# ChaissonLab/LRA

Hardware: AMD Instinct MI355X
Metric: aligned Gbp/s, 30 kb ONT vs GRCh38 (MapRead_lowacc end to end incl. SAM text), per job (higher is better)
Workload: dtype int32

## Files before the change

### lra_amd/csrc/indel_refine.hip

```cpp
#include "common.h"
#include "scan.h"
#include <algorithm>
#include <stdlib.h>

int lra_aog_launch_device(lra_ctx* ctx, int n, const char* d_qseq, const char* d_tseq, const uint64_t* d_q_off,
                          const int32_t* d_q_len, const uint64_t* d_t_off, const int32_t* d_t_len, const int32_t* d_k,
                          int m, int mm, int indel, int32_t* d_score, int32_t* d_nblocks, int32_t* d_blocks,
                          const uint64_t* d_block_off, int32_t* d_status);

namespace {

constexpr int BAD = -999999999;
constexpr int NEG = -2000000000;
enum { C_DIAG = 0, C_LEFT = 1, C_DOWN = 2, C_BOUND = 3, C_DELCLOSE = 4, C_INSCLOSE = 5, C_DONE = 6 };

__device__ __forceinline__ void wave_sync() {
  __builtin_amdgcn_fence(__ATOMIC_RELEASE, "workgroup");
  __builtin_amdgcn_wave_barrier();
  __builtin_amdgcn_fence(__ATOMIC_ACQUIRE, "workgroup");
}

__device__ __forceinline__ void wave_sync_lds() {
  __builtin_amdgcn_fence(__ATOMIC_RELEASE, "wavefront");
  __builtin_amdgcn_wave_barrier();
// ... 58 lines not shown
  auto get = [&](long i, long& q, long& t, long& l) {
    if (i == ovIdx) { q = ovQ; t = ovT; l = ovL; } else getRaw(i, q, t, l);
  };
  long startBlock = 0, endBlock = 0;
  while (endBlock < nB) {
    long q0, t0, l0;
    get(startBlock, q0, t0, l0);
    long qStart = q0, tStart = t0;
    long qPos = q0 + l0, tPos = t0 + l0;
    int tGap = 0, qGap = 0;
    long nq, nt, nl;
    if (endBlock < nB - 1) { get(endBlock + 1, nq, nt, nl); tGap = (int)(nt - tPos); qGap = (int)(nq - qPos); }
    long el = l0, eq = q0, et = t0;
    while (endBlock < nB - 1 && qGap < maxGap && tGap < maxGap && (startBlock == endBlock || el < 100)) {
      endBlock++;
      get(endBlock, eq, et, el);
      qPos = eq + el; tPos = et + el;
      if (endBlock + 1 < nB - 1) { get(endBlock + 1, nq, nt, nl); tGap = (int)(nt - tPos); qGap = (int)(nq - qPos); }
    }
    bool usedAlt = false;
    long altQ = 0, altT = 0, altL = 0;
    if (endBlock == startBlock) {
      pass(q0, t0, l0);
    } else {
      long fq = q0, ft = t0, fl = l0;
      if (l0 > maxGap) {
        long advanced = l0 - maxGap;
        pass(q0, t0, advanced);
        fq = q0 + advanced; ft = t0 + advanced; fl = maxGap;
        qStart += advanced; tStart += advanced;
      }
      long ll = el;
      if (el > maxGap) {
        usedAlt = true;
        altQ = eq + maxGap; altT = et + maxGap; altL = el - maxGap;
        ll = maxGap;
        qPos = eq + maxGap; tPos = et + maxGap;
      }
      const long qEnd = eq + ll, tEnd = et + ll;
      const long tLen = tPos - tStart;
      const long tSeqLen = tEnd - tStart, qSeqLen = qEnd - qStart;
      const bool aog = (tSeqLen < k || qSeqLen < k);
      if (EMIT) {
        const uint64_t s = so + nseg;
        A.s_aln[s] = a; A.s_kind[s] = aog ? 1 : 0;
        A.s_qStart[s] = (int)qStart; A.s_tStart[s] = (int)tStart; A.s_qEnd[s] = (int)qEnd; A.s_tEnd[s] = (int)tEnd;
        A.s_b0[s] = (int)startBlock; A.s_b1[s] = (int)endBlock;
        A.s_first[3 * s] = (int)fq; A.s_first[3 * s + 1] = (int)ft; A.s_first[3 * s + 2] = (int)fl;
        A.s_lastLen[s] = (int)ll;
        A.s_rows[s] = aog ? 0 : (uint64_t)(tLen > 0 ? tLen : 0);
        A.s_isAog[s] = aog ? 1u : 0u;
        A.i_kind[io + nitem] = 1; A.i_data[3 * (io + nitem)] = (int)(nseg);
      }
      nitem++; nseg++;
    }
    if (!usedAlt) endBlock++;
    else { ovIdx = endBlock; ovQ = altQ; ovT = altT; ovL = altL; }
    startBlock = endBlock;
  }
  if (!EMIT) { A.a_nseg[a] = nseg; A.a_nitem[a] = nitem; A.a_status[a] = 0; }
}

struct __attribute__((aligned(16))) Row { int S, E; unsigned int C; int T; };

constexpr int CB = 32;
constexpr int MAXW = 1024;

struct BandArgs {
  uint64_t n_seg, n_task;
  const int32_t* s_aln; const int32_t* s_kind; const int32_t* s_qStart; const int32_t* s_qEnd; const int32_t* s_tStart;
  const int32_t* s_b0; const int32_t* s_b1; const int32_t* s_first; const int32_t* s_lastLen;
  const uint64_t* s_rows; const uint64_t* s_row_off;
  const int32_t* ab; const uint64_t* block_off;
  const char* tseq; const uint64_t* t_off;
  int k;
  Row* rows;
  uint64_t* s_cells; int32_t* s_status; int32_t* s_width; uint64_t* s_tmpcap;
  uint32_t* s_nchunk; const uint64_t* chunk_off; uint32_t* task_seg; int32_t* chunkT; int32_t* chunkQ;
};

struct SegBlocks {
  const int32_t* ab; long b0, b1; int fq, ft, fl, lastLen;
  __device__ __forceinline__ void get(long b, long& q, long& t, long& l) const {
    if (b == b0) { q = fq; t = ft; l = fl; }
    else { q = ab[3 * b]; t = ab[3 * b + 1]; l = (b == b1) ? lastLen : ab[3 * b + 2]; }
  }
};
__device__ __forceinline__ SegBlocks seg_blocks(const BandArgs& B, uint64_t s) {
  SegBlocks v;
  const int a = B.s_aln[s];
  v.ab = B.ab + 3 * (B.block_off[a] + 2 * (uint64_t)a);
  v.b0 = B.s_b0[s]; v.b1 = B.s_b1[s];
  v.fq = B.s_first[3 * s]; v.ft = B.s_first[3 * s + 1]; v.fl = B.s_first[3 * s + 2]; v.lastLen = B.s_lastLen[s];
  return v;
}
struct BlockStep { int bqGap, btGap; long blockLength, rows, advq; };
__device__ __forceinline__ BlockStep block_step(const SegBlocks& sb, long b, long bq, long bt, long bl, long& nq2, long& nt2, long& nl2) {
  BlockStep st; st.bqGap = 0; st.btGap = 0; st.blockLength = bl; nq2 = nt2 = nl2 = 0;
  if (b < sb.b1) {
    sb.get(b + 1, nq2, nt2, nl2);
    st.bqGap = (int)(nq2 - (bq + bl)); st.btGap = (int)(nt2 - (bt + bl));
    if (st.bqGap > 0 && st.btGap > 0) { int c = min(st.bqGap, st.btGap); st.bqGap -= c; st.btGap -= c; st.blockLength += c; }
  }
  const long body = st.blockLength > 0 ? st.blockLength : 0;
  st.rows = body + (st.btGap > st.bqGap && st.btGap > 0 ? st.btGap : 0);
  st.advq = body + (st.bqGap > st.btGap && st.bqGap > 0 ? st.bqGap : 0);
  return st;
}

__global__ void ir_band_nchunk(BandArgs B) {
  const uint64_t s = (uint64_t)blockIdx.x * blockDim.x + threadIdx.x;
  if (s >= B.n_seg) return;
  B.s_nchunk[s] = (B.s_kind[s] != 0) ? 0u : (uint32_t)((B.s_b1[s] - B.s_b0[s] + 1 + CB - 1) / CB);
}
__global__ void ir_band_tasks(BandArgs B) {
  const uint64_t s = (uint64_t)blockIdx.x * blockDim.x + threadIdx.x;
  if (s >= B.n_seg) return;
  const uint64_t lo = B.chunk_off[s], hi = B.chunk_off[s + 1];
  for (uint64_t x = lo; x < hi; x++) B.task_seg[x] = (uint32_t)s;
  if (hi - lo <= 1) B.s_status[s] = 0;
}

__global__ void __launch_bounds__(64) ir_band_prep(BandArgs B) {
  const uint64_t s = blockIdx.x;
  const int lane = threadIdx.x;
  const uint64_t co = B.chunk_off[s];
  if (B.chunk_off[s + 1] - co <= 1) return;
  const SegBlocks sb = seg_blocks(B, s);
  const long nb = sb.b1 - sb.b0 + 1;
  long long carryT = 0, carryQ = 0;
  for (long base = 0; base < nb; base += 64) {
    const long i = base + lane;
    long long r = 0, q = 0;
    if (i < nb) {
      long bq, bt, bl, nq2, nt2, nl2;
      sb.get(sb.b0 + i, bq, bt, bl);
      const BlockStep st = block_step(sb, sb.b0 + i, bq, bt, bl, nq2, nt2, nl2);
      r = st.rows; q = st.advq;
    }
    long long ir = r, iq = q;
    for (int d = 1; d < 64; d <<= 1) {
      long long orr = __shfl_up(ir, d), oq = __shfl_up(iq, d);
      if (lane >= d) { ir += orr; iq += oq; }
    }
    if (i < nb && i > 0 && (i % CB) == 0) {
      B.chunkT[co + i / CB] = (int32_t)(carryT + ir - r);
      B.chunkQ[co + i / CB] = (int32_t)(sb.fq + carryQ + iq - q);
    }
    carryT += __shfl(ir, 63); carryQ += __shfl(iq, 63);
  }
  if (lane == 0) B.s_status[s] = (carryT != (long long)B.s_rows[s]) ? 1 : 0;
}

template <int RS>
__global__ void __launch_bounds__(64) ir_band_chunk(BandArgs B) {
  __shared__ int ringS[RS * 64], ringE[RS * 64];
  const int lane = threadIdx.x;
  const uint64_t x = (uint64_t)blockIdx.x * 64 + lane;
  if (x >= B.n_task) return;
  const uint64_t s = B.task_seg[x];
  const uint64_t co = B.chunk_off[s];
  const long c = (long)(x - co), nch = (long)(B.chunk_off[s + 1] - co);
  const bool multi = nch > 1, lastChunk = (c == nch - 1);
  if (multi && B.s_status[s] != 0) return;
  const long tLen = (long)B.s_rows[s];
  const SegBlocks sb = seg_blocks(B, s);
  const long qStart = B.s_qStart[s], qEnd = B.s_qEnd[s];
  const int k = B.k;
  Row* rows = B.rows + B.s_row_off[s];
  int status = 0;
#define RG(arr, r) arr[(int)((r) & (RS - 1)) * 64 + lane]
  for (int z = 0; z < RS; z++) { ringS[z * 64 + lane] = -1; ringE[z * 64 + lane] = -1; }
  const long bFirst = sb.b0 + c * CB, bLast = min(sb.b1, bFirst + CB - 1);
  const long T0 = c > 0 ? B.chunkT[co + c] : 0;
  long from = c;
  while (from > 0) { from--; if (from == 0 || T0 - B.chunkT[co + from] >= 2 * (long)k - 1) break; }
  const long ownLo = c > 0 ? T0 - k + 1 : 0, thr = T0 - 2 * (long)k + 1;
  long q = from > 0 ? B.chunkQ[co + from] : sb.fq;
  long tOff = from > 0 ? B.chunkT[co + from] : 0;
  auto flush = [&](long r) {
    if (r >= 0 && r < tLen) {
      if (r >= ownLo) { int2 v; v.x = RG(ringS, r); v.y = RG(ringE, r); *(int2*)&rows[r] = v; }
      RG(ringS, r) = -1; RG(ringE, r) = -1;
    }
  };
  long bq, bt, bl;
  sb.get(sb.b0 + from * CB, bq, bt, bl);
  bool live = (c == 0);
  int eMin = -1;
  long sHi = -1;
  for (long b = sb.b0 + from * CB; b <= bLast && !(status & 1); b++) {
    long nq2, nt2, nl2;
    const BlockStep st = block_step(sb, b, bq, bt, bl, nq2, nt2, nl2);
    if (!live) {
      if (b < bFirst && tOff + st.rows <= thr) { tOff += st.rows; q += st.advq; bq = nq2; bt = nt2; bl = nl2; continue; }
      live = true;
    }
    for (long bi = 0; bi < st.blockLength; bi++) {
      if (tOff >= tLen) { status |= 1; break; }
      int newE;
      {
        int lo = (int)max(q - k, qStart);
        int cs = RG(ringS, tOff), ce = RG(ringE, tOff);
        RG(ringS, tOff) = (cs == -1) ? lo : min(cs, lo);
        newE = ce;
        if (ce == -1 || ce < q + k) { newE = (int)min(qEnd - 1, q + k); RG(ringE, tOff) = newE; }
      }
      if (newE < eMin) eMin = newE;
      if (q > eMin) {
        int m = 0x7fffffff;
        for (int ki = 0; ki < k; ki++)
          if (tOff - ki >= 0) { int e = RG(ringE, tOff - ki); if (e < q) { e = (int)q; RG(ringE, tOff - ki) = e; } m = min(m, e); }
        eMin = m;
      }
      if (sHi < tOff) sHi = tOff;
      for (long r = sHi + 1; r <= tOff + k - 1 && r < tLen; r++) RG(ringS, r) = (int)q;
      if (sHi < tOff + k - 1) sHi = tOff + k - 1;
      tOff++; q++;
      flush(tOff - k);
    }
    if (st.bqGap > st.btGap) {
      for (int qi = 0; qi < st.bqGap; qi++, q++)
        for (int ki = 0; ki < k; ki++) {
          if (tOff - ki >= 0 && tOff - ki < tLen) { if (RG(ringE, tOff - ki) < q) RG(ringE, tOff - ki) = (int)q; }
          if (tOff + ki < tLen) { int v = RG(ringS, tOff + ki); if (v == 0 || v > q) RG(ringS, tOff + ki) = (int)q; }
        }
    }
    if (st.btGap > st.bqGap) {
      for (int ti = 0; ti < st.btGap; ti++) {
        if (tOff >= tLen) { status |= 1; break; }
        const int e = (int)min(qEnd - 1, q + k);
        RG(ringS, tOff) = (int)max(q - k, qStart); RG(ringE, tOff) = e;
        if (e < eMin) eMin = e;
        if (sHi < tOff) sHi = tOff;
        tOff++;
        flush(tOff - k);
      }
    }
    bq = nq2; bt = nt2; bl = nl2;
  }
  if (lastChunk) for (long r = max(0L, tOff - k + 1); r < tLen; r++) flush(r);
#undef RG
  if (!multi) { if (tOff != tLen) status |= 1; B.s_status[s] = status; }
}

__global__ void __launch_bounds__(64) ir_band_scan(BandArgs B) {
  const uint64_t s = blockIdx.x;
  const int lane = threadIdx.x;
  if (B.s_kind[s] != 0) { if (lane == 0) { B.s_cells[s] = 0; B.s_status[s] = 0; B.s_width[s] = 0; B.s_tmpcap[s] = 0; } return; }
  int status = B.s_status[s];
  const long tLen = (long)B.s_rows[s];
  Row* rows = B.rows + B.s_row_off[s];
  unsigned long long cells = 0;
  int width = 0;
  if (!status && tLen > 0) {
    int run = 0x7fffffff;
    for (long base = ((tLen - 1) / 64) * 64; base >= 0; base -= 64) {
      const long r = base + lane;
      const int own = (r < tLen) ? rows[r].S : 0x7fffffff;
      int v = own;
      for (int d = 1; d < 64; d <<= 1) { int o = __shfl_down(v, d); if (lane + d < 64) v = min(v, o); }
      v = min(v, run);
      if (r < tLen && v != own) rows[r].S = v;
      run = __shfl(v, 0);
    }
    const int a = B.s_aln[s];
    const unsigned char* tb = (const unsigned char*)B.tseq + B.t_off[a] + B.s_tStart[s];
    int runE = -0x7fffffff;
    for (long base = 0; base < tLen; base += 64) {
      const long r = base + lane;
      Row w; w.S = 0; w.E = -0x7fffffff; w.C = 0; w.T = 0;
      if (r < tLen) w = rows[r];
      int e = w.E;
      for (int d = 1; d < 64; d <<= 1) { int o = __shfl_up(e, d); if (lane >= d) e = max(e, o); }
      e = max(e, runE);
      runE = __shfl(e, 63);
      int len = (r < tLen) ? e - w.S + 1 : 0;
      if (r < tLen) {
        if (len < 1 || w.S < 0) status |= 1;
        else if (len > MAXW) status |= 4;
        width = max(width, len);
      }
      const unsigned long long l = (unsigned long long)max(len, 0);
      unsigned long long inc = l;
      for (int d = 1; d < 64; d <<= 1) { unsigned long long o = __shfl_up(inc, d); if (lane >= d) inc += o; }
      if (r < tLen) { w.E = e; w.C = (unsigned int)(cells + inc - l); w.T = tb[r]; rows[r] = w; }
      cells += __shfl(inc, 63);
    }
    for (int o = 32; o > 0; o >>= 1) { status |= __shfl_xor(status, o); width = max(width, __shfl_xor(width, o)); }
  }
  if (lane == 0) {
    B.s_cells[s] = status ? 0 : cells;
    B.s_status[s] = status;
    B.s_width[s] = status ? 0 : width;
    B.s_tmpcap[s] = status ? 0 : (uint64_t)(tLen + ((long)B.s_qEnd[s] - B.s_qStart[s]) + 2);
  }
}

constexpr int FILL_BINS = 128;
template <bool EMIT>
__global__ void ir_classify(uint64_t n_seg, const int32_t* __restrict__ s_kind, const int32_t* __restrict__ s_status, const int32_t* __restrict__ s_width,
                            const uint64_t* __restrict__ s_rows, int* bins, uint32_t* list) {
  const uint64_t s = (uint64_t)blockIdx.x * blockDim.x + threadIdx.x;
  const int lane = threadIdx.x & 63;
  int bin = -1;
  if (s < n_seg && s_kind[s] == 0 && s_status[s] == 0) {
    const int w = s_width[s];
    const uint32_t r = (uint32_t)min((unsigned long long)s_rows[s], 0x7fffffffULL);
    bin = (w <= 16 ? 0 : w <= 32 ? 1 : w <= 64 ? 2 : 3) * 32 + (r ? __clz(r) : 31);
  }
  const unsigned long long below = (lane == 0) ? 0ULL : (~0ULL >> (64 - lane));
  unsigned long long todo = __ballot(bin >= 0);
  while (todo) {
    const int leader = __ffsll((long long)todo) - 1;
    const int b = __shfl(bin, leader);
    const unsigned long long m = __ballot(bin == b);
    int base = 0;
    if (lane == leader) base = atomicAdd(&bins[b], __popcll(m));
    base = __shfl(base, leader);
    if (EMIT && bin == b) list[base + __popcll(m & below)] = (uint32_t)s;
    todo &= ~m;
  }
}

struct FillArgs {
  uint64_t n_seg;
  const int32_t* s_aln; const uint64_t* s_rows; const uint64_t* s_row_off; const uint64_t* s_cell_off;
  const Row* rows;
  const char* qseq; const uint64_t* q_off; const int32_t* q_len;
  int match, mismatch, g;
  unsigned char* path;
  const uint32_t* list; int* cursor;
};

__device__ __forceinline__ bool is_bound(long row, int c, int len) { return c == len - 1 || (row > 0 && c == 0); }

__device__ __forceinline__ int shr1(int x, int fill) { return __builtin_amdgcn_update_dpp(fill, x, 0x138, 0xf, 0xf, false); }
template <int G>
__device__ __forceinline__ int scan_max(int w) {
  w = max(w, __builtin_amdgcn_update_dpp(NEG, w, 0x111, 0xf, 0xf, false));
  w = max(w, __builtin_amdgcn_update_dpp(NEG, w, 0x112, 0xf, 0xf, false));
  w = max(w, __builtin_amdgcn_update_dpp(NEG, w, 0x114, 0xf, 0xf, false));
  w = max(w, __builtin_amdgcn_update_dpp(NEG, w, 0x118, 0xf, 0xf, false));
  if (G >= 32) w = max(w, __builtin_amdgcn_update_dpp(NEG, w, 0x142, 0xa, 0xf, false));
  if (G >= 64) w = max(w, __builtin_amdgcn_update_dpp(NEG, w, 0x143, 0xc, 0xf, false));
  return w;
}

template <int G>
__global__ void __launch_bounds__(64) ir_fill(FillArgs F) {
  constexpr int GP = 64 / G;
  constexpr int CLS = (G == 16) ? 0 : (G == 32) ? 1 : 2;
  const int lane = threadIdx.x;
  const int c = lane % G, gbase = lane - c;
  const int g = F.g, go = 2 * F.g + 1;
  const long listEnd = F.cursor[4 + CLS];
  const uint32_t* list = F.list;
  long ti = -1, tLen = 0;
  const Row* rows = nullptr; const unsigned char* qb = nullptr; unsigned char* P = nullptr;
  long chunkBase = 0, qLast = 0;
  Row chunk; chunk.S = chunk.E = chunk.T = 0; chunk.C = 0;
  int W0 = 0, qlo = 0, qhi = 0, qnext = 0;
  int prevM = BAD, prevD = BAD, prevS = 0, prevLen = 0;
  bool done = false;
  auto ldq = [&](long idx) -> int { return qb[idx < qLast ? idx : qLast]; };
  while (true) {
    if (!done && ti < 0) {
      long x = 0;
      if (c == 0) x = atomicAdd(&F.cursor[CLS], 1);
      x = __shfl(x, gbase);
      if (x < listEnd) {
        const uint64_t s = list[x];
        const int a = F.s_aln[s];
        tLen = (long)F.s_rows[s];
        rows = F.rows + F.s_row_off[s];
        qb = (const unsigned char*)F.qseq + F.q_off[a];
        qLast = (long)F.q_len[a] - 1;
        P = F.path + F.s_cell_off[s];
        ti = 0; chunkBase = 0;
        if (c < tLen) chunk = rows[c];
        W0 = rows[0].S;
        qlo = ldq((long)W0 + c); qhi = ldq((long)W0 + G + c); qnext = ldq((long)W0 + 2 * G + c);
      } else done = true;
    }
    if (__ballot(!done) == 0ULL) break;
    if (!done && ti - chunkBase == G) { chunkBase = ti; if (ti + c < tLen) chunk = rows[ti + c]; }
    const int src = gbase + (int)((ti - chunkBase) & (G - 1));
    const int S = __shfl(chunk.S, src), E = __shfl(chunk.E, src), tch = __shfl(chunk.T, src);
    const unsigned int C = __shfl(chunk.C, src);
    while (!done && S - W0 >= G) { W0 += G; qlo = qhi; qhi = qnext; qnext = ldq((long)W0 + 2 * G + c); }
    const int j = S - W0 + c;
    const int q1 = __shfl(qlo, gbase + (j & (G - 1))), q2 = __shfl(qhi, gbase + (j & (G - 1)));
    const int qch = (j < G) ? q1 : q2;
    const int len = E - S + 1;
    const bool lastRow = (ti == tLen - 1);
    const int off = S - prevS;
// ... 460 lines not shown
  int st = 0;
  for (uint64_t s = seg_off[a]; s < seg_off[a + 1]; s++) {
    if (s_kind[s] == 0) { int x = s_status[s]; if (x & 1) st |= LRA_ST_OOB_SLOT; if (x & 2) st |= LRA_ST_NO_TERMINATION; if (x & 4) st |= LRA_ST_RANGE; }
    else st |= p_status[s_aog_idx[s]];
  }
  a_status[a] = st;
}

__global__ void ir_item_aln(int n_aln, const uint64_t* item_off, int32_t* i_aln) {
  int a = blockIdx.x * blockDim.x + threadIdx.x;
  if (a >= n_aln) return;
  for (uint64_t i = item_off[a]; i < item_off[a + 1]; i++) i_aln[i] = a;
}

__global__ void ir_aog_setup(uint64_t n_seg, const int32_t* s_kind, const int32_t* s_aln, const uint64_t* s_aog_off ,
                             const int32_t* s_qStart, const int32_t* s_tStart, const int32_t* s_qEnd, const int32_t* s_tEnd,
                             const uint64_t* q_off, const uint64_t* t_off, int k, uint32_t* s_aog_idx, uint64_t* p_q_off, int32_t* p_q_len,
                             uint64_t* p_t_off, int32_t* p_t_len, int32_t* p_k, uint32_t* p_cap) {
  uint64_t s = (uint64_t)blockIdx.x * blockDim.x + threadIdx.x;
  if (s >= n_seg) return;
  if (s_kind[s] != 1) { s_aog_idx[s] = 0; return; }
  uint32_t p = (uint32_t)s_aog_off[s];
  s_aog_idx[s] = p;
  int a = s_aln[s];
  p_q_off[p] = q_off[a] + (uint64_t)s_qStart[s]; p_q_len[p] = s_qEnd[s] - s_qStart[s];
  p_t_off[p] = t_off[a] + (uint64_t)s_tStart[s]; p_t_len[p] = s_tEnd[s] - s_tStart[s];
  p_k[p] = k;
  p_cap[p] = (uint32_t)(min(p_q_len[p], p_t_len[p]) + 1);
}


struct Arena {
  char* base; size_t cap, used;
  template <typename T> T* get(size_t n) {
    size_t bytes = (n * sizeof(T) + 255) & ~(size_t)255;
    if (used + bytes > cap) return nullptr;
    T* p = (T*)(base + used);
    used += bytes;
    return p;
  }
};

}

template <typename CT>
static void scan(lra_ctx* ctx, long n, const CT* c, uint64_t* off) {
  (void)lra_exclusive_scan<CT>(ctx, n, c, off);
}

static int d2h(lra_ctx* ctx, void* dst, const void* src, size_t bytes) {
  LRA_HIP_CHECK(ctx, hipMemcpyAsync(dst, src, bytes, hipMemcpyDeviceToHost, ctx->stream));
  LRA_HIP_CHECK(ctx, hipStreamSynchronize(ctx->stream));
  return LRA_OK;
}

extern "C" int lra_indel_refine_batch(lra_ctx* ctx, int n_aln, const int32_t* d_blocks_in, const uint64_t* d_block_off, uint64_t n_blocks_in,
                                      const char* d_qseq, const uint64_t* d_q_off, const int32_t* d_q_len, const char* d_tseq,
                                      const uint64_t* d_t_off, const int64_t* d_t_len, int refine_band, int match, int mismatch,
                                      int indel, int end_align, lra_refine_result* out) {
  if (!ctx || !out || n_aln < 0) return LRA_ERR_INVALID;
  if (refine_band < 2 || refine_band > 64) return lra_set_err(ctx, LRA_ERR_INVALID, "refine_band must be 2..64");
  if (indel >= 0) return lra_set_err(ctx, LRA_ERR_INVALID, "indel score must be negative");
  memset(out, 0, sizeof(*out));
  if (n_aln == 0) return LRA_OK;
  LRA_HIP_CHECK(ctx, hipSetDevice(ctx->device));
  hipStream_t st = ctx->stream;
  const size_t nA = (size_t)n_aln, nBk = (size_t)n_blocks_in + 2 * nA;
  const size_t perAln = ((nA * 4 + 255) & ~(size_t)255) * 3 + (((nA + 1) * 8 + 255) & ~(size_t)255) * 3;
  char* baseP = (char*)lra_ensure(ctx, 70, perAln + 4096);
  if (!baseP) return LRA_ERR_NOMEM;
  Arena ap{baseP, perAln + 4096, 0};
  IRArgs A;
  memset(&A, 0, sizeof A);
  A.n_aln = n_aln; A.blocks_in = d_blocks_in; A.block_off = d_block_off;
  A.qseq = d_qseq; A.q_off = d_q_off; A.q_len = d_q_len; A.tseq = d_tseq; A.t_off = d_t_off; A.t_len = d_t_len;
  A.k = refine_band; A.match = match; A.mismatch = mismatch; A.indel = indel; A.endAlign = end_align;
  A.a_nseg = ap.get<uint32_t>(nA); A.a_nitem = ap.get<uint32_t>(nA); A.a_status = ap.get<int32_t>(nA);
  uint64_t* seg_off = ap.get<uint64_t>(nA + 1); uint64_t* item_off = ap.get<uint64_t>(nA + 1); uint64_t* out_block_off = ap.get<uint64_t>(nA + 1);
  if (!out_block_off) return lra_set_err(ctx, LRA_ERR_NOMEM, "arena accounting");
  A.seg_off = seg_off; A.item_off = item_off;
  const int nbA = (n_aln + SEG_LANES - 1) / SEG_LANES;
  lra_time_begin(ctx, "ir_segment");
  hipLaunchKernelGGL(ir_segment<false>, dim3(nbA), dim3(64), 0, st, A);
  lra_time_end(ctx);
  scan(ctx, (long)n_aln, A.a_nseg, seg_off);
  scan(ctx, (long)n_aln, A.a_nitem, item_off);
  uint64_t n_seg = 0, n_item = 0;
  if (d2h(ctx, &n_seg, seg_off + n_aln, 8) || d2h(ctx, &n_item, item_off + n_aln, 8)) return LRA_ERR_HIP;
  const size_t capSeg = (size_t)n_seg + 1, capItem = (size_t)n_item + 1;
  size_t needA = 0;
  auto add = [&](size_t n, size_t sz) { needA += ((n * sz + 255) & ~(size_t)255); };
  add(3 * nBk, 4);
  for (int i = 0; i < 8; i++) add(capSeg, 4);
  add(3 * capSeg, 4); add(capSeg, 4); add(capSeg, 8); add(capSeg, 4);
  add(capSeg + 1, 8); add(capSeg + 1, 8); add(capSeg, 8); add(capSeg + 1, 8); add(capSeg, 4);
  add(capSeg, 4); add(capSeg, 4); add(capSeg, 8); add(capSeg + 1, 8); add(capSeg, 4); add(capSeg + 1, 8);
  add(capSeg, 4); add(FILL_BINS + 8, 4);
  add(capItem, 4); add(3 * capItem, 4); add(capItem, 4); add(capItem, 4); add(capItem + 1, 8);
  add(capSeg, 8); add(capSeg, 4); add(capSeg, 8); add(capSeg, 4); add(capSeg, 4); add(capSeg, 4); add(capSeg + 1, 8);
  add(capSeg, 4); add(capSeg, 4); add(capSeg, 4);
  add(capSeg, 4); add(capSeg + 1, 8);
  char* baseA = (char*)lra_scratch(ctx, 2, needA + 4096);
  if (!baseA) return LRA_ERR_NOMEM;
  Arena ar{baseA, needA + 4096, 0};
  A.ab = ar.get<int32_t>(3 * nBk);
  A.s_aln = ar.get<int32_t>(capSeg); A.s_kind = ar.get<int32_t>(capSeg); A.s_qStart = ar.get<int32_t>(capSeg); A.s_tStart = ar.get<int32_t>(capSeg);
  A.s_qEnd = ar.get<int32_t>(capSeg); A.s_tEnd = ar.get<int32_t>(capSeg); A.s_b0 = ar.get<int32_t>(capSeg); A.s_b1 = ar.get<int32_t>(capSeg);
  A.s_first = ar.get<int32_t>(3 * capSeg); A.s_lastLen = ar.get<int32_t>(capSeg); A.s_rows = ar.get<uint64_t>(capSeg); A.s_isAog = ar.get<uint32_t>(capSeg);
  uint64_t* s_row_off = ar.get<uint64_t>(capSeg + 1); uint64_t* s_aog_off = ar.get<uint64_t>(capSeg + 1);
  uint64_t* s_cells = ar.get<uint64_t>(capSeg); uint64_t* s_cell_off = ar.get<uint64_t>(capSeg + 1); int32_t* s_status = ar.get<int32_t>(capSeg);
  uint32_t* s_nblk = ar.get<uint32_t>(capSeg); int32_t* s_width = ar.get<int32_t>(capSeg); uint64_t* s_tmpcap = ar.get<uint64_t>(capSeg);
  uint64_t* s_tmp_off = ar.get<uint64_t>(capSeg + 1); uint32_t* s_aog_idx = ar.get<uint32_t>(capSeg); uint64_t* s_out_off = ar.get<uint64_t>(capSeg + 1);
  uint32_t* fill_lists = ar.get<uint32_t>(capSeg); int* fill_counts = ar.get<int>(FILL_BINS + 8);
  A.i_kind = ar.get<int32_t>(capItem); A.i_data = ar.get<int32_t>(3 * capItem);
  int32_t* i_aln = ar.get<int32_t>(capItem); uint32_t* i_count = ar.get<uint32_t>(capItem); uint64_t* i_out_off = ar.get<uint64_t>(capItem + 1);
  uint64_t* p_q_off = ar.get<uint64_t>(capSeg); int32_t* p_q_len = ar.get<int32_t>(capSeg); uint64_t* p_t_off = ar.get<uint64_t>(capSeg);
  int32_t* p_t_len = ar.get<int32_t>(capSeg); int32_t* p_k = ar.get<int32_t>(capSeg); uint32_t* p_cap = ar.get<uint32_t>(capSeg);
  uint64_t* p_block_off = ar.get<uint64_t>(capSeg + 1);
  int32_t* p_score = ar.get<int32_t>(capSeg); int32_t* p_nblocks = ar.get<int32_t>(capSeg); int32_t* p_status = ar.get<int32_t>(capSeg);
  uint32_t* s_nchunk = ar.get<uint32_t>(capSeg); uint64_t* chunk_off = ar.get<uint64_t>(capSeg + 1);
  if (!chunk_off) return lra_set_err(ctx, LRA_ERR_NOMEM, "arena accounting");
  lra_time_begin(ctx, "ir_segment");
  hipLaunchKernelGGL(ir_segment<true>, dim3(nbA), dim3(64), 0, st, A);
  lra_time_end(ctx);
  hipLaunchKernelGGL(ir_item_aln, dim3((n_aln + 255) / 256), dim3(256), 0, st, n_aln, item_off, i_aln);
  uint64_t n_rows = 0, n_aog = 0, n_cells = 0;
  const int32_t* tmp_blocks = nullptr;
  if (n_seg) {
    scan(ctx, (long)n_seg, A.s_rows, s_row_off);
    scan(ctx, (long)n_seg, A.s_isAog, s_aog_off);
    if (d2h(ctx, &n_rows, s_row_off + n_seg, 8) || d2h(ctx, &n_aog, s_aog_off + n_seg, 8)) return LRA_ERR_HIP;
    Row* rows = (Row*)lra_ensure(ctx, 0, (n_rows + 1) * sizeof(Row));
    if (!rows) return LRA_ERR_NOMEM;
    BandArgs B;
    B.n_seg = n_seg; B.s_aln = A.s_aln; B.s_kind = A.s_kind; B.s_qStart = A.s_qStart; B.s_qEnd = A.s_qEnd; B.s_tStart = A.s_tStart;
    B.s_b0 = A.s_b0; B.s_b1 = A.s_b1; B.s_first = A.s_first; B.s_lastLen = A.s_lastLen; B.s_rows = A.s_rows; B.s_row_off = s_row_off;
    B.ab = A.ab; B.block_off = d_block_off; B.tseq = d_tseq; B.t_off = d_t_off; B.k = refine_band; B.rows = rows;
    B.s_cells = s_cells; B.s_status = s_status; B.s_width = s_width; B.s_tmpcap = s_tmpcap;
    const unsigned gridL = (unsigned)((n_seg + 63) / 64);
    const unsigned gridS = (unsigned)((n_seg + 255) / 256);
    lra_time_begin(ctx, "ir_band");
    B.s_nchunk = s_nchunk; B.chunk_off = chunk_off; B.n_task = 0; B.task_seg = nullptr; B.chunkT = nullptr; B.chunkQ = nullptr;
    hipLaunchKernelGGL(ir_band_nchunk, dim3(gridS), dim3(256), 0, st, B);
    scan(ctx, (long)n_seg, s_nchunk, chunk_off);
    uint64_t n_task = 0;
    if (d2h(ctx, &n_task, chunk_off + n_seg, 8)) return LRA_ERR_HIP;
    uint32_t* task_seg = (uint32_t*)lra_ensure(ctx, 54, (n_task + 1) * 4);
    int32_t* chunk_tq = (int32_t*)lra_ensure(ctx, 55, (n_task + 1) * 8);
    if (!task_seg || !chunk_tq) return LRA_ERR_NOMEM;
    B.n_task = n_task; B.task_seg = task_seg; B.chunkT = chunk_tq; B.chunkQ = chunk_tq + n_task + 1;
    hipLaunchKernelGGL(ir_band_tasks, dim3(gridS), dim3(256), 0, st, B);
    hipLaunchKernelGGL(ir_band_prep, dim3((unsigned)n_seg), dim3(64), 0, st, B);
    if (n_task) {
      const unsigned gridT = (unsigned)((n_task + 63) / 64);
      if (refine_band <= 8) hipLaunchKernelGGL(ir_band_chunk<16>, dim3(gridT), dim3(64), 0, st, B);
      else if (refine_band <= 32) hipLaunchKernelGGL(ir_band_chunk<64>, dim3(gridT), dim3(64), 0, st, B);
      else hipLaunchKernelGGL(ir_band_chunk<128>, dim3(gridT), dim3(64), 0, st, B);
    }
    hipLaunchKernelGGL(ir_band_scan, dim3((unsigned)n_seg), dim3(64), 0, st, B);
    lra_time_end(ctx);
    scan(ctx, (long)n_seg, s_cells, s_cell_off);
    scan(ctx, (long)n_seg, s_tmpcap, s_tmp_off);
    uint64_t n_tmp = 0;
    if (d2h(ctx, &n_cells, s_cell_off + n_seg, 8) || d2h(ctx, &n_tmp, s_tmp_off + n_seg, 8)) return LRA_ERR_HIP;
    const size_t pathBytes = (n_cells + 256 + 255) & ~(size_t)255;
    unsigned char* path = (unsigned char*)lra_ensure(ctx, 12, pathBytes + (n_tmp + 1) * 12 + 256);
    if (!path) return LRA_ERR_NOMEM;
    int32_t* tmpb = (int32_t*)(path + pathBytes);
    tmp_blocks = tmpb;
    int h_bins[FILL_BINS], h_start[FILL_BINS], h_cursor[8] = {0, 0, 0, 0, 0, 0, 0, 0};
    LRA_HIP_CHECK(ctx, hipMemsetAsync(fill_counts, 0, FILL_BINS * 4, st));
    hipLaunchKernelGGL(ir_classify<false>, dim3((unsigned)((n_seg + 255) / 256)), dim3(256), 0, st, n_seg, A.s_kind, s_status, s_width, A.s_rows, fill_counts, fill_lists);
    if (d2h(ctx, h_bins, fill_counts, FILL_BINS * 4)) return LRA_ERR_HIP;
    { int run = 0; for (int b = 0; b < FILL_BINS; b++) { h_start[b] = run; run += h_bins[b]; if ((b & 31) == 0) h_cursor[b / 32] = h_start[b]; if ((b & 31) == 31) h_cursor[4 + b / 32] = run; } }
    LRA_HIP_CHECK(ctx, hipMemcpyAsync(fill_counts, h_start, FILL_BINS * 4, hipMemcpyHostToDevice, st));
    hipLaunchKernelGGL(ir_classify<true>, dim3((unsigned)((n_seg + 255) / 256)), dim3(256), 0, st, n_seg, A.s_kind, s_status, s_width, A.s_rows, fill_counts, fill_lists);
    int* fill_cursor = fill_counts + FILL_BINS;
    LRA_HIP_CHECK(ctx, hipMemcpyAsync(fill_cursor, h_cursor, 32, hipMemcpyHostToDevice, st));
    FillArgs F;
    F.n_seg = n_seg; F.s_aln = A.s_aln; F.s_rows = A.s_rows; F.s_row_off = s_row_off; F.s_cell_off = s_cell_off; F.rows = rows;
    F.qseq = d_qseq; F.q_off = d_q_off; F.q_len = d_q_len; F.match = match; F.mismatch = mismatch; F.g = indel; F.path = path;
    F.list = fill_lists; F.cursor = fill_cursor;
    const unsigned cap_grid = (unsigned)ctx->num_cu * 32;
    if (getenv("LRA_IR_DBG")) {
      const int hc[4] = {h_cursor[4] - h_cursor[0], h_cursor[5] - h_cursor[1], h_cursor[6] - h_cursor[2], h_cursor[7] - h_cursor[3]};
      fprintf(stderr, "[ir] n_seg %llu n_rows %llu n_cells %llu n_task %llu n_item %llu fill classes 16/32/64/wide: %d %d %d %d\n",
              (unsigned long long)n_seg, (unsigned long long)n_rows, (unsigned long long)n_cells, (unsigned long long)n_task,
              (unsigned long long)n_item, hc[0], hc[1], hc[2], hc[3]);
    }
    lra_time_begin(ctx, "ir_fill");
    const uint64_t n16 = (uint64_t)(h_cursor[4] - h_cursor[0]), n32 = (uint64_t)(h_cursor[5] - h_cursor[1]), n64 = (uint64_t)(h_cursor[6] - h_cursor[2]);
    const uint64_t nWide = (uint64_t)(h_cursor[7] - h_cursor[3]);
    if (n16) hipLaunchKernelGGL(ir_fill_cols<1>, dim3((unsigned)std::min<uint64_t>((n16 + 3) / 4, cap_grid)), dim3(64), 0, lra_side_fork(ctx, 1), F);
    if (n64) hipLaunchKernelGGL(ir_fill<64>, dim3((unsigned)std::min<uint64_t>(n64, cap_grid)), dim3(64), 0, lra_side_fork(ctx, 2), F);
    if (nWide) hipLaunchKernelGGL(ir_fill_wide, dim3((unsigned)std::min<uint64_t>(nWide, cap_grid)), dim3(64), 0, lra_side_fork(ctx, 3), F);
    if (n32) hipLaunchKernelGGL(ir_fill_cols<2>, dim3((unsigned)std::min<uint64_t>((n32 + 3) / 4, cap_grid)), dim3(64), 0, st, F);
    if (n16) lra_side_join(ctx, 1);
    if (n64) lra_side_join(ctx, 2);
    if (nWide) lra_side_join(ctx, 3);
    lra_time_end(ctx);
    TraceArgs T;
    T.n_seg = n_seg; T.s_kind = A.s_kind; T.s_tStart = A.s_tStart; T.s_rows = A.s_rows; T.s_row_off = s_row_off;
    T.s_cells = s_cells; T.s_cell_off = s_cell_off; T.s_status = s_status; T.rows = rows; T.path = path;
    T.s_nblk = s_nblk; T.s_tmp_off = s_tmp_off; T.tmp_blocks = tmpb;
    lra_time_begin(ctx, "ir_trace");
    hipLaunchKernelGGL(ir_trace_wave, dim3((unsigned)n_seg), dim3(64), 0, st, T);
    lra_time_end(ctx);
    if (n_aog) {
      hipLaunchKernelGGL(ir_aog_setup, dim3((unsigned)((n_seg + 255) / 256)), dim3(256), 0, st, n_seg, A.s_kind, A.s_aln, s_aog_off, A.s_qStart,
                         A.s_tStart, A.s_qEnd, A.s_tEnd, d_q_off, d_t_off, refine_band, s_aog_idx, p_q_off, p_q_len, p_t_off, p_t_len, p_k, p_cap);
      scan(ctx, (long)n_aog, p_cap, p_block_off);
      uint64_t aog_cap = 0;
      if (d2h(ctx, &aog_cap, p_block_off + n_aog, 8)) return LRA_ERR_HIP;
      if (aog_cap * 12 + 64 > ctx->aux_bytes) {
        if (ctx->aux) (void)hipFree(ctx->aux);
        ctx->aux = nullptr; ctx->aux_bytes = 0;
        size_t want = aog_cap * 12 + aog_cap * 3 + 4096;
        if (hipMalloc(&ctx->aux, want) != hipSuccess) return lra_set_err(ctx, LRA_ERR_NOMEM, "aog block buffer");
        ctx->aux_bytes = want;
      }
      int rc = lra_aog_launch_device(ctx, (int)n_aog, d_qseq, d_tseq, p_q_off, p_q_len, p_t_off, p_t_len, p_k, match, mismatch, indel, p_score,
                                     p_nblocks, (int32_t*)ctx->aux, p_block_off, p_status);
      if (rc) return rc;
    }
  }
  hipLaunchKernelGGL(ir_item_counts, dim3((unsigned)((n_item + 255) / 256)), dim3(256), 0, st, n_item, A.i_kind, A.i_data, i_aln, seg_off, A.s_kind,
                     s_nblk, s_aog_idx, p_nblocks, i_count);
  scan(ctx, (long)n_item, i_count, i_out_off);
  uint64_t n_out = 0;
  if (d2h(ctx, &n_out, i_out_off + n_item, 8)) return LRA_ERR_HIP;
  if ((n_out + 1) * 12 > ctx->out_bytes) {
    if (ctx->out_buf) (void)hipFree(ctx->out_buf);
    ctx->out_buf = nullptr; ctx->out_bytes = 0;
    size_t want = (n_out + 1) * 12 + (n_out + 1) * 3 + 4096;
    if (hipMalloc(&ctx->out_buf, want) != hipSuccess) return lra_set_err(ctx, LRA_ERR_NOMEM, "refined block buffer");
    ctx->out_bytes = want;
  }
  int32_t* out_blocks = (int32_t*)ctx->out_buf;
  hipLaunchKernelGGL(ir_finalize_offsets, dim3((unsigned)((std::max<uint64_t>(n_item, nA + 1) + 255) / 256)), dim3(256), 0, st, n_aln, n_item, item_off,
                     i_out_off, A.i_kind, A.i_data, i_aln, seg_off, s_out_off, out_block_off);
  GatherArgs G;
  G.n_item = n_item; G.i_kind = A.i_kind; G.i_data = A.i_data; G.i_aln = i_aln; G.i_out_off = i_out_off; G.seg_off = seg_off;
  G.s_kind = A.s_kind; G.s_qStart = A.s_qStart; G.s_tStart = A.s_tStart; G.s_aog_idx = s_aog_idx;
  G.aog_blocks = (const int32_t*)ctx->aux; G.aog_block_off = p_block_off; G.aog_nblocks = p_nblocks;
  G.tmp_blocks = tmp_blocks; G.s_tmp_off = s_tmp_off; G.s_nblk = s_nblk; G.out_blocks = out_blocks;
  lra_time_begin(ctx, "ir_gather");
  if (n_item) hipLaunchKernelGGL(ir_gather, dim3((unsigned)std::min<uint64_t>(n_item, 65535 * 4)), dim3(64), 0, st, G);
  lra_time_end(ctx);
  hipLaunchKernelGGL(ir_aln_status, dim3((n_aln + 255) / 256), dim3(256), 0, st, n_aln, seg_off, A.s_kind, s_status, s_aog_idx, p_status, A.a_status);
  LRA_HIP_CHECK(ctx, hipGetLastError());
  LRA_HIP_CHECK(ctx, hipStreamSynchronize(st));
  out->n_aln = n_aln; out->n_blocks = n_out; out->n_segments = n_seg; out->n_cells = n_cells; out->n_rows = n_rows; out->n_aog = n_aog;
  out->d_block_off = out_block_off; out->d_blocks = out_blocks; out->d_status = A.a_status;
  return LRA_OK;
}
```

Before: 1.086.

## Compute refine band rows in parallel per wavefront instead of serial ring simulation

Replaces the one-thread-per-chunk sequential ring-buffer band simulation with a kernel that gives each chunk a full wavefront. The wavefront stages block prefix offsets in LDS using DPP scans and expands them into a per-row event ring. Each lane then derives its row's band start and end directly from a window of neighbouring events, with a fallback that walks blocks from global memory. The aim is to remove long serial per-thread loops and their divergence, at the cost of more complex windowing logic, redundant per-row window work, and a risk of semantic mismatch with the old band construction.

```diff
diff --git a/lra_amd/csrc/indel_refine.hip b/lra_amd/csrc/indel_refine.hip
--- a/lra_amd/csrc/indel_refine.hip
+++ b/lra_amd/csrc/indel_refine.hip
@@ -234,96 +234,219 @@
   if (lane == 0) B.s_status[s] = (carryT != (long long)B.s_rows[s]) ? 1 : 0;
 }
 
-template <int RS>
-__global__ void __launch_bounds__(64) ir_band_chunk(BandArgs B) {
-  __shared__ int ringS[RS * 64], ringE[RS * 64];
+constexpr int TR = 64;
+constexpr int NB = 256;
+constexpr int EV = 256;
+
+__device__ __forceinline__ int step_gap(const BlockStep& st) {
+  return (st.bqGap > st.btGap && st.bqGap > 0) ? st.bqGap : (st.btGap > st.bqGap && st.btGap > 0) ? -st.btGap : 0;
+}
+__device__ __forceinline__ int wave_scan_add(int w) {
+  w += __builtin_amdgcn_update_dpp(0, w, 0x111, 0xf, 0xf, false);
+  w += __builtin_amdgcn_update_dpp(0, w, 0x112, 0xf, 0xf, false);
+  w += __builtin_amdgcn_update_dpp(0, w, 0x114, 0xf, 0xf, false);
+  w += __builtin_amdgcn_update_dpp(0, w, 0x118, 0xf, 0xf, false);
+  w += __builtin_amdgcn_update_dpp(0, w, 0x142, 0xa, 0xf, false);
+  w += __builtin_amdgcn_update_dpp(0, w, 0x143, 0xc, 0xf, false);
+  return w;
+}
+__device__ __forceinline__ void band_query_gap(int& S, int q0, int G) {
+  if (S == 0 || S > q0) S = q0;
+  if (G >= 2 && S == 0) S = q0 + 1;
+}
+
+__device__ __forceinline__ int band_after(int2 e) { return e.x + (e.y == 1 ? 1 : 0); }
+__device__ __forceinline__ int2 band_row_ring(const int2* ev, int r, int k, int tLen, int qStart, int qEnd, int fq) {
+  int S = -1, E = -1;
+  const int x0 = max(r - k + 1, 0), x1 = min(r + k - 1, tLen);
+  for (int x = x0; x < r; x++) {
+    const int2 e = ev[x & (EV - 1)];
+    if (e.y == 1) { S = e.x; break; }
+  }
+  if (S == 0) {
+    int cnt = x0 > 0 ? band_after(ev[(x0 - 1) & (EV - 1)]) : fq;
+    S = -1;
+    for (int x = x0; x < r; x++) {
+      const int2 e = ev[x & (EV - 1)];
+      if (e.x > cnt) band_query_gap(S, cnt, e.x - cnt);
+      if (e.y == 1 && (S == -1 || S > e.x)) S = e.x;
+      cnt = band_after(e);
+    }
+  }
+  const int cnt = r > 0 ? band_after(ev[(r - 1) & (EV - 1)]) : fq;
+  const int2 e = ev[r & (EV - 1)];
+  const int q = e.x;
+  if (q > cnt) { E = q - 1; band_query_gap(S, cnt, q - cnt); }
+  const int lo = max(q - k, qStart), hi = min(qEnd - 1, q + k);
+  if (e.y == 0) { S = lo; E = hi; }
+  else if (e.y == 1) {
+    S = (S == -1) ? lo : min(S, lo);
+    if (E == -1 || E < q + k) E = hi;
+    if (E < q) E = q;
+    if (S == -1 || S > q) S = q;
+  }
+  const int last = band_after(ev[x1 & (EV - 1)]);
+  if (last > band_after(e)) E = max(E, last - 1);
+  return make_int2(S, E);
+}
+
+struct BandGlobalCur {
+  const SegBlocks* sb; long b, bLimit; int adv;
+  int T, Q, body, G, end; bool valid;
+  __device__ __forceinline__ void load() {
+    valid = b <= bLimit;
+    if (valid) {
+      long bq, bt, bl, n1, n2, n3;
+      sb->get(b, bq, bt, bl);
+      const BlockStep st = block_step(*sb, b, bq, bt, bl, n1, n2, n3);
+      body = (int)(st.blockLength > 0 ? st.blockLength : 0); G = step_gap(st); end = T + (int)st.rows; adv = (int)st.advq;
+    }
+  }
+  __device__ __forceinline__ void seek(int x0) { load(); while (valid && end < x0) next(); }
+  __device__ __forceinline__ void next() { T = end; Q += adv; b++; load(); }
+};
+__device__ __forceinline__ int2 band_row_blocks(BandGlobalCur& cu, int r, int k, int tLen, int qStart, int qEnd) {
+  int S = -1, E = -1;
+  const int x0 = max(r - k + 1, 0), x1 = min(r + k - 1, tLen);
+  cu.seek(x0);
+  for (int x = x0; x <= x1; x++) {
+    while (cu.valid && cu.end == x) {
+      if (cu.G > 0) {
+        const int q0 = cu.Q + cu.body;
+        if (x >= r && E < q0 + cu.G - 1) E = q0 + cu.G - 1;
+        if (x <= r) band_query_gap(S, q0, cu.G);
+      }
+      cu.next();
+    }
+    if (x < tLen && cu.valid) {
+      const int d = x - cu.T;
+      const bool gapRow = d >= cu.body;
+      const int q = cu.Q + (gapRow ? cu.body : d);
+      if (x == r) {
+        const int lo = max(q - k, qStart), hi = min(qEnd - 1, q + k);
+        if (gapRow) { S = lo; E = hi; }
+        else {
+          S = (S == -1) ? lo : min(S, lo);
+          if (E == -1 || E < q + k) E = hi;
+          if (E < q) E = q;
+          if (S == -1 || S > q) S = q;
+        }
+      } else if (!gapRow) {
+        if (x > r) { if (E < q) E = q; }
+        else if (S == -1 || S > q) S = q;
+      }
+    }
+  }
+  return make_int2(S, E);
+}
+
+__global__ void __launch_bounds__(64) ir_band_rows(BandArgs B) {
+  __shared__ int LT[NB + 1], LQ[NB + 1];
+  __shared__ int2 ev[EV];
   const int lane = threadIdx.x;
-  const uint64_t x = (uint64_t)blockIdx.x * 64 + lane;
-  if (x >= B.n_task) return;
+  const uint64_t x = blockIdx.x;
   const uint64_t s = B.task_seg[x];
   const uint64_t co = B.chunk_off[s];
   const long c = (long)(x - co), nch = (long)(B.chunk_off[s + 1] - co);
   const bool multi = nch > 1, lastChunk = (c == nch - 1);
   if (multi && B.s_status[s] != 0) return;
-  const long tLen = (long)B.s_rows[s];
+  const int tLen = (int)B.s_rows[s];
   const SegBlocks sb = seg_blocks(B, s);
-  const long qStart = B.s_qStart[s], qEnd = B.s_qEnd[s];
+  const int qStart = B.s_qStart[s], qEnd = B.s_qEnd[s];
   const int k = B.k;
   Row* rows = B.rows + B.s_row_off[s];
-  int status = 0;
-#define RG(arr, r) arr[(int)((r) & (RS - 1)) * 64 + lane]
-  for (int z = 0; z < RS; z++) { ringS[z * 64 + lane] = -1; ringE[z * 64 + lane] = -1; }
-  const long bFirst = sb.b0 + c * CB, bLast = min(sb.b1, bFirst + CB - 1);
-  const long T0 = c > 0 ? B.chunkT[co + c] : 0;
+  const long bLimit = min(sb.b1, sb.b0 + c * CB + CB - 1);
+  const int T0 = c > 0 ? B.chunkT[co + c] : 0;
   long from = c;
-  while (from > 0) { from--; if (from == 0 || T0 - B.chunkT[co + from] >= 2 * (long)k - 1) break; }
-  const long ownLo = c > 0 ? T0 - k + 1 : 0, thr = T0 - 2 * (long)k + 1;
-  long q = from > 0 ? B.chunkQ[co + from] : sb.fq;
-  long tOff = from > 0 ? B.chunkT[co + from] : 0;
-  auto flush = [&](long r) {
-    if (r >= 0 && r < tLen) {
-      if (r >= ownLo) { int2 v; v.x = RG(ringS, r); v.y = RG(ringE, r); *(int2*)&rows[r] = v; }
-      RG(ringS, r) = -1; RG(ringE, r) = -1;
-    }
+  while (from > 0) { from--; if (from == 0 || T0 - B.chunkT[co + from] >= 2 * k - 1) break; }
+  const int ownLo = c > 0 ? max(T0 - k + 1, 0) : 0;
+  const int ownHi = lastChunk ? tLen : min(max(B.chunkT[co + c + 1] - k + 1, 0), tLen);
+  long sB = sb.b0 + from * CB;
+  int sT = from > 0 ? B.chunkT[co + from] : 0, sQ = from > 0 ? B.chunkQ[co + from] : sb.fq;
+  int n = 0, bt = sT, bq = sQ;
+  long b = sB;
+  auto stage = [&]() {
+    n = 0; bt = sT; bq = sQ; b = sB;
+    while (n < NB && b <= bLimit) {
+      int r = 0, a = 0;
+      if (b + lane <= bLimit) {
+        long q_, t_, l_, n1, n2, n3;
+        sb.get(b + lane, q_, t_, l_);
+        const BlockStep st = block_step(sb, b + lane, q_, t_, l_, n1, n2, n3);
+        r = (int)st.rows; a = (int)st.advq;
+      }
+      const int ir = wave_scan_add(r), ia = wave_scan_add(a);
+      const int cnt = (int)min(64L, bLimit - b + 1);
+      if (lane < cnt) { LT[n + lane] = bt + ir - r; LQ[n + lane] = bq + ia - a; }
+      bt += __builtin_amdgcn_readlane(ir, cnt - 1); bq += __builtin_amdgcn_readlane(ia, cnt - 1);
+      n += cnt; b += cnt;
+    }
+    if (lane == 0) { LT[n] = bt; LQ[n] = bq; }
+    wave_sync_lds();
   };
-  long bq, bt, bl;
-  sb.get(sb.b0 + from * CB, bq, bt, bl);
-  bool live = (c == 0);
-  int eMin = -1;
-  long sHi = -1;
-  for (long b = sb.b0 + from * CB; b <= bLast && !(status & 1); b++) {
-    long nq2, nt2, nl2;
-    const BlockStep st = block_step(sb, b, bq, bt, bl, nq2, nt2, nl2);
-    if (!live) {
-      if (b < bFirst && tOff + st.rows <= thr) { tOff += st.rows; q += st.advq; bq = nq2; bt = nt2; bl = nl2; continue; }
-      live = true;
-    }
-    for (long bi = 0; bi < st.blockLength; bi++) {
-      if (tOff >= tLen) { status |= 1; break; }
-      int newE;
-      {
-        int lo = (int)max(q - k, qStart);
-        int cs = RG(ringS, tOff), ce = RG(ringE, tOff);
-        RG(ringS, tOff) = (cs == -1) ? lo : min(cs, lo);
-        newE = ce;
-        if (ce == -1 || ce < q + k) { newE = (int)min(qEnd - 1, q + k); RG(ringE, tOff) = newE; }
-      }
-      if (newE < eMin) eMin = newE;
-      if (q > eMin) {
-        int m = 0x7fffffff;
-        for (int ki = 0; ki < k; ki++)
-          if (tOff - ki >= 0) { int e = RG(ringE, tOff - ki); if (e < q) { e = (int)q; RG(ringE, tOff - ki) = e; } m = min(m, e); }
-        eMin = m;
-      }
-      if (sHi < tOff) sHi = tOff;
-      for (long r = sHi + 1; r <= tOff + k - 1 && r < tLen; r++) RG(ringS, r) = (int)q;
-      if (sHi < tOff + k - 1) sHi = tOff + k - 1;
-      tOff++; q++;
-      flush(tOff - k);
-    }
-    if (st.bqGap > st.btGap) {
-      for (int qi = 0; qi < st.bqGap; qi++, q++)
-        for (int ki = 0; ki < k; ki++) {
-          if (tOff - ki >= 0 && tOff - ki < tLen) { if (RG(ringE, tOff - ki) < q) RG(ringE, tOff - ki) = (int)q; }
-          if (tOff + ki < tLen) { int v = RG(ringS, tOff + ki); if (v == 0 || v > q) RG(ringS, tOff + ki) = (int)q; }
+  stage();
+  if (!multi) {
+    const int status = (bt != tLen) ? 1 : 0;
+    if (lane == 0) B.s_status[s] = status;
+    if (status) return;
+  }
+  int evHi = 0;
+  for (int lo = ownLo; lo < ownHi;) {
+    int hi = min(lo + TR, ownHi);
+    { const int e0 = max(evHi, max(lo - k, 0)); if (e0 + 65 - k > lo) hi = min(hi, e0 + 65 - k); }
+    const int xmax = min(hi + k - 2, tLen);
+    bool fresh = false;
+    if (!(b > bLimit || bt > xmax) && n > 0) {
+      fresh = true;
+      const int xn = max(lo - k, 0);
+      int first = n;
+      for (int j = 0; j < n; j += 64) {
+        const unsigned long long m = __ballot(j + lane < n && LT[min(j + lane, n - 1) + 1] >= xn);
+        if (m) { first = j + __ffsll((long long)m) - 1; break; }
+      }
+      if (first < n) { sT = __builtin_amdgcn_readfirstlane(LT[first]); sQ = __builtin_amdgcn_readfirstlane(LQ[first]); } else { sT = bt; sQ = bq; }
+      sB += first;
+      wave_sync_lds();
+      stage();
+    }
+    const bool covered = b > bLimit || bt > xmax;
+    if (!covered) hi = min(hi, bt - k + 1);
+    if (hi <= lo && !fresh) continue;
+    const int r = lo + lane;
+    if (hi > lo) {
+      const int needHi = min(hi + k - 2, tLen);
+      evHi = max(evHi, max(lo - k, 0));
+      wave_sync_lds();
+      for (; evHi <= needHi; evHi += 64) {
+        const int xx = evHi + lane;
+        if (xx <= needHi) {
+          int l = 0, h = n;
+          while (l < h) { const int mid = (l + h) >> 1; if (LT[mid + 1] > xx) h = mid; else l = mid + 1; }
+          int2 e = make_int2(LQ[n], 2);
+          if (l < n && xx < tLen) {
+            const int t0 = LT[l], q0 = LQ[l];
+            const int d = xx - t0, body = min(LT[l + 1] - t0, LQ[l + 1] - q0);
+            if (d >= 0) e = make_int2(q0 + min(d, body), d < body ? 1 : 0);
+          }
+          ev[xx & (EV - 1)] = e;
         }
-    }
-    if (st.btGap > st.bqGap) {
-      for (int ti = 0; ti < st.btGap; ti++) {
-        if (tOff >= tLen) { status |= 1; break; }
-        const int e = (int)min(qEnd - 1, q + k);
-        RG(ringS, tOff) = (int)max(q - k, qStart); RG(ringE, tOff) = e;
-        if (e < eMin) eMin = e;
-        if (sHi < tOff) sHi = tOff;
-        tOff++;
-        flush(tOff - k);
-      }
-    }
-    bq = nq2; bt = nt2; bl = nl2;
-  }
-  if (lastChunk) for (long r = max(0L, tOff - k + 1); r < tLen; r++) flush(r);
-#undef RG
-  if (!multi) { if (tOff != tLen) status |= 1; B.s_status[s] = status; }
+      }
+      evHi = needHi + 1;
+      wave_sync_lds();
+      if (r < hi) {
+        const int2 w = band_row_ring(ev, r, k, tLen, qStart, qEnd, (int)sb.fq);
+        *(int4*)&rows[r] = make_int4(w.x, w.y, 0, 0);
+      }
+    } else {
+      hi = min(lo + TR, ownHi);
+      if (r < hi) {
+        BandGlobalCur cu; cu.sb = &sb; cu.b = sB; cu.bLimit = bLimit; cu.T = sT; cu.Q = sQ;
+        const int2 w = band_row_blocks(cu, r, k, tLen, qStart, qEnd);
+        *(int4*)&rows[r] = make_int4(w.x, w.y, 0, 0);
+      }
+    }
+    lo = hi;
+  }
 }
 
 __global__ void __launch_bounds__(64) ir_band_scan(BandArgs B) {
@@ -1090,10 +1213,7 @@
     hipLaunchKernelGGL(ir_band_tasks, dim3(gridS), dim3(256), 0, st, B);
     hipLaunchKernelGGL(ir_band_prep, dim3((unsigned)n_seg), dim3(64), 0, st, B);
     if (n_task) {
-      const unsigned gridT = (unsigned)((n_task + 63) / 64);
-      if (refine_band <= 8) hipLaunchKernelGGL(ir_band_chunk<16>, dim3(gridT), dim3(64), 0, st, B);
-      else if (refine_band <= 32) hipLaunchKernelGGL(ir_band_chunk<64>, dim3(gridT), dim3(64), 0, st, B);
-      else hipLaunchKernelGGL(ir_band_chunk<128>, dim3(gridT), dim3(64), 0, st, B);
+      hipLaunchKernelGGL(ir_band_rows, dim3((unsigned)n_task), dim3(64), 0, st, B);
     }
     hipLaunchKernelGGL(ir_band_scan, dim3((unsigned)n_seg), dim3(64), 0, st, B);
     lra_time_end(ctx);
```

Result: no change. 1.094 (median of 5 runs) (+0.7%).
